# Lqm26/BMCNet-ESR

Measured on AMD Instinct MI355X. Metric: LR-voxel-frames/sec x4 SR train step, NFS-shaped 180x240 (BASELINE configs[1] / [2]), f32, higher is better.
Workload: dtype f32; 1 GPU; BMCNet(scale=4, n_c=128, n_b=5) x4 SR train step, NFS-shaped 180x240 (BASELINE configs[1] / [2]) -> 720x960, bs=4/GPU, arithmetic fp32 (native fp32 MFMA; 3x3 convolutions through Winograd F(4x4,3x3) / F(2x2,3x3) transforms in fp32), SEQL=9 SEQN=2 (8 windows BPTT), event scatter + fwd + MSE + bwd + Adam(amsgrad); global_batch=4, parallelism=dp1, rccl_ranks=1, rccl_initialised_before_headline_run=False

## Files before the change

### bmcnet-esr_amd/bmc_hip/ops.py

```python
from __future__ import annotations

import ctypes as C
import os
import threading
import weakref
from typing import List, Optional, Sequence

import torch

from . import lib

CK = 16
_cur_dev = torch._C._cuda_getDevice


_STREAM_OVERRIDE = None
_STREAM_OVERRIDE_TS = None


def _stream():
    if _STREAM_OVERRIDE is not None:
        return _STREAM_OVERRIDE
    return torch._C._cuda_getCurrentRawStream(_cur_dev())

# ... 302 lines not shown
    G, Cout, Cin, taps = w4.shape
    if wino:
        npos = 36 if wino == 4 else 16
        hit = _cache_get(spec, ("fw", npos), owner)
        if hit is not None:
            return hit
        cp = coutpad(Cout)
        out = torch.empty(G * spec.kpad * npos * cp, device=w4.device, dtype=torch.float32)
        fn, nm = (lib._pack_wino4, "bmc_pack_weight_wino4") if wino == 4 else (lib._pack_wino, "bmc_pack_weight_wino")
        lib.call(fn, nm, w4.data_ptr(), spec.kmap(w4.device).data_ptr(), G, Cout, Cin,
                 spec.kpad, cp, 0, 0, 0, out.data_ptr(), _stream())
        _cache_put(spec, ("fw", npos), owner, out)
        return out
    hit = _cache_get(spec, ("f", MATH), owner)
    if hit is not None:
        return hit
    cp = coutpad(Cout)
    out = torch.empty(G * spec.kpad * taps * cp, device=w4.device, dtype=torch.float32)
    lib.call(lib._pack_w, "bmc_pack_weight", w4.data_ptr(), spec.kmap(w4.device).data_ptr(), G, Cout, Cin, taps,
             spec.kpad, cp, out.data_ptr(), _stream())
    if MATH:
        out = _split_planes(out, cp)
    _cache_put(spec, ("f", MATH), owner, out)
    return out


def _packed_weight_t(w4: torch.Tensor, spec: ConvSpec, src_index: int, owner, wino=False):
    G, Cout, Cin, taps = w4.shape
    k0 = sum(spec.nch[:src_index])
    nk = spec.nch[src_index]
    nkpad = coutpad(nk)
    c16 = round_up(Cout, CK)
    if wino:
        npos = 36 if wino == 4 else 16
        hit = _cache_get(spec, ("tw", src_index, npos), owner)
        if hit is not None:
            return hit
        out = torch.empty(G * c16 * npos * nkpad, device=w4.device, dtype=torch.float32)
        fn, nm = (lib._pack_wino4, "bmc_pack_weight_wino4") if wino == 4 else (lib._pack_wino, "bmc_pack_weight_wino")
        lib.call(fn, nm, w4.data_ptr(), spec.kmap(w4.device).data_ptr(), G, Cout, Cin,
                 c16, nkpad, 1, k0, nk, out.data_ptr(), _stream())
        _cache_put(spec, ("tw", src_index, npos), owner, out)
        return out
    hit = _cache_get(spec, ("t", src_index, MATH), owner)
    if hit is not None:
        return hit
    out = torch.empty(G * c16 * taps * nkpad, device=w4.device, dtype=torch.float32)
    lib.call(lib._pack_wt, "bmc_pack_weight_t", w4.data_ptr(), spec.kmap(w4.device).data_ptr(), G, Cout, Cin, taps,
             k0, nk, nkpad, c16, out.data_ptr(), _stream())
    if MATH:
        out = _split_planes(out, nkpad)
    _cache_put(spec, ("t", src_index, MATH), owner, out)
    return out



def conv_raw(srcs: List[lib.Src], wpacked, w_group_stride, bias, bias_group_stride, out_ptr, out_batch_stride,
             out_pix_stride, B, H, W, Cout, taps, relu=False, residual: Optional[lib.Src] = None, bpg=None,
             accumulate=False, flops=0.0, mask: Optional[lib.Src] = None, wino=False):
    a = lib.ConvArgs()
    a.nsrc = len(srcs)
    for i, s in enumerate(srcs):
        a.src[i] = s
    a.wpacked = wpacked.data_ptr()
    a.bias = bias.data_ptr() if bias is not None else None
    a.w_group_stride = w_group_stride * MATH // 2 if MATH else w_group_stride
    a.math = MATH
    if wino:
        assert MATH == 0 and taps == 9
        a.w_group_stride = w_group_stride // 9 * (36 if wino == 4 else 16)
        a.math = 5 if wino == 4 else 4
    a.bias_group_stride = bias_group_stride
    a.batch_per_group = bpg if bpg else B
    a.out = out_ptr
    a.out_batch_stride = out_batch_stride
    a.out_pix_stride = out_pix_stride
    a.B, a.H, a.W = B, H, W
    a.Cout, a.Coutpad = Cout, coutpad(Cout)
    a.taps = taps
    a.relu = int(relu)
    a.residual = residual if residual is not None else _null_src()
    a.mask = mask if mask is not None else _null_src()
    a.accumulate = int(accumulate)
    e0 = _prof_begin()
    lib.call(lib._conv, "bmc_conv", C.byref(a), _stream())
    _prof_end(e0, ("wino4_conv<9,128>" if wino == 4 else "wino_conv<9,128>") if wino else
              "conv_kernel<%d,%d>" % (taps, 32 if a.Coutpad == 32 else 128), flops,
              4.0 * B * H * W * (sum(x.nch for x in srcs) + Cout * (1 + (residual is not None) + (mask is not None) + bool(accumulate))))
    if PROFILE is not None and e0 is not None:
        PROFILE_WINO[0 if wino else 1] += 1


_ZEROS = {}


def _zeros(device):
    z = _ZEROS.get(device)
    if z is None:
        z = torch.zeros(64, device=device, dtype=torch.float32)
        _ZEROS[device] = z
    return z


TAP_SPLIT_TILES = 8


def pgemm_raw(a_src: lib.Src, srcs: List[lib.Src], B, H, W, taps, bpg, M, N, device, flops=0.0, want_bias=False):
    G = B // bpg
    mpad, npad = round_up(M, 32), round_up(N, 32)
    if taps == 9:
        cols = 32 if MATH == 3 else 64
        n_nblk = (npad + cols - 1) // cols
        tiles = ((H + 3) // 4) * ((W + 15) // 16)
        target = 256
    else:
        n_nblk = (npad + 127) // 128
        tiles = (H * W + 63) // 64
        target = 256
    other = G * ((mpad + 127) // 128) * n_nblk
    nsplit = max(1, min(bpg * tiles, target // max(other, 1)))
    tap_groups = 1
    if taps == 9 and MATH in (0, 1) and bpg * tiles < TAP_SPLIT_TILES * nsplit and nsplit >= 3:
        tap_groups = 3
        nsplit = max(1, min(bpg * tiles, target // max(other * 3, 1)))
    slabs = torch.empty(nsplit * G * taps * mpad * npad, device=device, dtype=torch.float32)
    p = lib.PgemmArgs()
    p.a = a_src
    p.nsrc = len(srcs)
    for i, s in enumerate(srcs):
        p.src[i] = s
    p.B, p.H, p.W, p.taps = B, H, W, taps
    p.batch_per_group = bpg
    p.slabs = slabs.data_ptr()
    p.nsplit = nsplit
    p.zeros = _zeros(device).data_ptr()
    p.math = MATH
    p.tap_groups = tap_groups
    bslabs = None
    if want_bias:
        bslabs = torch.empty(nsplit * G * 4 * mpad, device=device, dtype=torch.float32)
        p.bias_slabs = bslabs.data_ptr()
    else:
        p.bias_slabs = None
    _on_side(slabs, bslabs)
    e0 = _prof_begin()
    lib.call(lib._pgemm, "bmc_pgemm", C.byref(p), _stream())
    _prof_end(e0, "pgemm_kernel<%d>" % taps, flops, 4.0 * B * H * W * (a_src.nch + sum(x.nch for x in srcs)) + 4.0 * slabs.numel())
    if want_bias:
        return slabs, nsplit, G, bslabs
    return slabs, nsplit, G


WINO_WGRAD = os.environ.get("BMC_WINO_WGRAD", "1") != "0"
WINO4_WGRAD = os.environ.get("BMC_WINO4_WGRAD", "0") != "0"
WINO4_WGRAD_MIN_STAGES = int(os.environ.get("BMC_WINO4_WGRAD_MIN_STAGES", 24))


def wgrad_wino4_ok(B, H, W):
    if not WINO4_WGRAD:
        return False
    stages = B * ((H + 3) // 4) * (((W + 3) // 4 + 3) // 4)
    return stages >= 32 * WINO4_WGRAD_MIN_STAGES


def wino_wgrad_ok(a_src, x_srcs, spec, taps, Cout, G):
    if not (WINO and WINO_WGRAD and MATH == 0 and taps == 9 and G == 1 and Cout == 128 and len(x_srcs) == 1 and spec.kpad == 128):
        return False
    xs = x_srcs[0]
    if not (xs.nch == 128 and xs.pix_stride == 128 and a_src.nch == 128 and a_src.pix_stride == 128):
        return False
    k0 = spec.kmap_host[0]
    return k0 >= 0 and spec.kmap_host == list(range(k0, k0 + 128))


WGRAD_MERGE = max(1, min(8, int(os.environ.get("BMC_WGRAD_MERGE", 5))))
WGRAD_MERGE_MAX_PIXELS = int(os.environ.get("BMC_WGRAD_MERGE_MAX_PIXELS", 1 << 17))


_WINDOW = [0]


def next_window():
    _WINDOW[0] += 1
    return _WINDOW[0]


def current_window():
    return _WINDOW[0]


class _MergeQueue:
    __slots__ = ("items", "spec", "dev", "w_param", "b_param", "want_bias", "k0", "full", "H", "W", "window", "pg")

    def __init__(self, spec, dev, w_param, b_param, want_bias, k0, full, H, W, window, pg=None):
        self.items = []
        self.spec, self.dev, self.w_param, self.b_param, self.want_bias, self.k0, self.full, self.H, self.W, self.window, self.pg = \
            spec, dev, w_param, b_param, want_bias, k0, full, H, W, window, pg


_MERGE = {}
_FLUSH_QUEUED = set()
PTR_TABLE_MAX = 256


def flush_wgrads(task=None):
    if task is None:
        task = torch._C._current_graph_task_id()
    _FLUSH_QUEUED.discard(task)
    qs = _MERGE.pop(task, None)
    if not qs:
        return
    for q in list(qs.values()):
        if q.items:
            _launch_merged(q)


def _queue_flush(task):
    if task not in _FLUSH_QUEUED:
        _FLUSH_QUEUED.add(task)
        torch.autograd.Variable._execution_engine.queue_callback(lambda: flush_wgrads(task))


_TABLES = {}


def _table_src(srcs, batches, btot, dev):
    ptrs = []
    for s_, nb in zip(srcs, batches):
        mod = s_.batch_mod if s_.batch_mod >= 1 else 1
        ptrs.extend(s_.ptr + 4 * (((i + s_.batch_shift) % mod) * s_.batch_stride) for i in range(nb))
    st = _stream()
    key = (dev.index, st.value if hasattr(st, "value") else st, tuple(ptrs))
    table = _TABLES.get(key)
    if table is None:
        if len(_TABLES) >= 8192:
            _TABLES.clear()
        table = torch.empty(btot, device=dev, dtype=torch.int64)
        lib.call(lib._ptr_table, "bmc_ptr_table", (C.c_ulonglong * btot)(*ptrs), btot, table.data_ptr(), st)
        if not torch.cuda.is_current_stream_capturing():
            _TABLES[key] = table
    t = lib.Src()
    t.ptr = table.data_ptr()
    t.batch_stride, t.pix_stride, t.nch, t.batch_shift, t.batch_mod = 0, srcs[0].pix_stride, srcs[0].nch, 0, -1
    return t, table


def _launch_merged(q):
    items, q.items = q.items, []
    keep = tuple(t for it in items for t in it[3])
    npx = items[0][2] * q.H * q.W
    if q.pg is not None:
        taps, Cout, w_shape = q.pg
        batches = [it[2] for it in items]
        btot = sum(batches)
        nx = len(items[0][1])
        with wgrad_side(npx, [q.w_param, q.b_param] if q.want_bias else [q.w_param], keep):
            a_t, tab_a = _table_src([it[0] for it in items], batches, btot, q.dev)
            x_tt = [_table_src([it[1][k] for it in items], batches, btot, q.dev) for k in range(nx)]
            x_t = [t for t, _ in x_tt]
            _on_side(tab_a, *[tb for _, tb in x_tt])
            r = pgemm_raw(a_t, x_t, btot, q.H, q.W, taps, btot, Cout, q.spec.kpad, q.dev,
                          flops=2.0 * btot * q.H * q.W * Cout * taps * q.spec.kreal, want_bias=q.want_bias)
            reduce_wgrad(r[0], r[1], 1, taps, Cout, q.spec, q.dev, r[3] if q.want_bias else None, q.w_param,
                         q.b_param if q.want_bias else None, w_shape)
        return
    with wgrad_side(npx, [q.w_param, q.b_param] if q.want_bias else [q.w_param], keep):
        _wgrad_wino([it[0] for it in items], [it[1] for it in items], [it[2] for it in items], q.H, q.W, q.spec, q.dev, q.w_param,
                    q.b_param, None, q.want_bias, q.k0, q.full)


def _queue_use(key, make_queue, item, task, npx):
    qs = _MERGE.setdefault(task, {})
    q = qs.get(key)
    if q is None or q.w_param is not item[4] or q.window != item[5]:
        if q is not None and q.items:
            _launch_merged(q)
        q = qs[key] = make_queue()
    if q.pg is not None and q.items and sum(it[2] for it in q.items) + item[2] > PTR_TABLE_MAX:
        _launch_merged(q)
    _queue_flush(task)
    _side_arm(npx)
    q.items.append(item[:4])
    if len(q.items) >= WGRAD_MERGE:
        _launch_merged(q)


def _mergeable(B, H, W, w_param, b_param, want_bias, keep, window):
    task = torch._C._current_graph_task_id()
    ok = (WGRAD_MERGE > 1 and window is not None and B * H * W <= WGRAD_MERGE_MAX_PIXELS and task >= 0 and w_param is not None
          and not isinstance(w_param, (tuple, list)) and is_sink(w_param) and (not want_bias or is_sink(b_param)) and keep
          and not torch.cuda.is_current_stream_capturing())
    return ok, task


def wgrad_pgemm(a_src, x_srcs, B, H, W, taps, Cout, spec, dev, w_param, b_param, w_shape, G=1, want_bias=True, keep=(), window=None):
    if G == 1:
        ok, task = _mergeable(B, H, W, w_param, b_param, want_bias, keep, window)
        if ok and B <= PTR_TABLE_MAX and all(x.batch_mod != -1 for x in x_srcs) and a_src.batch_mod != -1:
            key = (id(w_param), "pg", taps, len(x_srcs), H, W, bool(want_bias))
            _queue_use(key, lambda: _MergeQueue(spec, dev, w_param, b_param, want_bias, None, spec.covers_all, H, W, window,
                                                pg=(taps, Cout, w_shape)),
                       (a_src, list(x_srcs), B, tuple(keep), w_param, window), task, B * H * W)
            return None, None
    with wgrad_side(B * H * W, _flat_params(w_param, b_param if want_bias else None), keep):
        r = pgemm_raw(a_src, x_srcs, B, H, W, taps, B // G, Cout, spec.kpad, dev, flops=2.0 * B * H * W * Cout * taps * spec.kreal,
                      want_bias=want_bias)
        return reduce_wgrad(r[0], r[1], G, taps, Cout, spec, dev, r[3] if want_bias else None, w_param,
# ... 1056 lines not shown
```

### bmcnet-esr_amd/csrc/wino4_wgrad.hip

```cpp
#include "bmc_common.h"
#include "dma_ring.h"
#include <stdlib.h>

#ifndef BMC_W4G_ABL
#define BMC_W4G_ABL 0
#endif

#ifdef BMC_W4G_STAMP
__device__ unsigned long long g_w4g_stamp[8][64][8];
#define W4G_STAMP(it, k) do { if (blockIdx.x == 8 && (threadIdx.x & 63) == 0 && (it) >= 40 && (it) < 104) g_w4g_stamp[threadIdx.x >> 6][(it) - 40][(k)] = __builtin_amdgcn_s_memtime(); } while (0)
#else
#define W4G_STAMP(it, k) do { } while (0)
#endif

namespace {

struct Wgrad4K {
    SrcDev a;
    SrcDev x;
    int B, H, W;
    int TY, SX;
    int nstages, nsplit;
    float* part;
    float* bias_part;
};

typedef float f32x2 __attribute__((ext_vector_type(2)));

__device__ __forceinline__ const float* uni(const float* p) {
    const unsigned long long v = reinterpret_cast<unsigned long long>(p);
    const unsigned lo = __builtin_amdgcn_readfirstlane((unsigned)v), hi = __builtin_amdgcn_readfirstlane((unsigned)(v >> 32));
    return reinterpret_cast<const float*>(((unsigned long long)hi << 32) | lo);
}

constexpr int NPW = 18;
constexpr int TS = 4;
constexpr int CH = 64;
constexpr int PIMG = TS * CH;
constexpr int IMG = NPW * PIMG;
constexpr int SIMG = 2 * IMG;
constexpr int XPC = 23, YPC = 16;
constexpr int RAWX = XPC * 256;
constexpr int RAWF = (XPC + YPC) * 256;
constexpr int NPC = XPC + YPC;
constexpr int PPW = 10;
constexpr int LDSF = 2 * RAWF + 2 * SIMG;

template <int TG>
__device__ __forceinline__ void wgrad4_body(const Wgrad4K& a, float* const lds, const int split, const int chh, const int kh) {
    const int tid = threadIdx.x, lane = tid & 63;
    const int wave = __builtin_amdgcn_readfirstlane(tid >> 6);
    float* const rawb = lds;
    float* const imgb = lds + 2 * RAWF;
    const unsigned lds_raw = (unsigned)(size_t)(__attribute__((address_space(3))) void*)rawb;

    const int pg = wave >> 2, cb = (wave >> 1) & 1, kb = wave & 1;
    const int l31 = lane & 31, lh = lane >> 5;
    const int aoff = 3 * pg * PIMG + lh * CH + 32 * cb + l31;
    const int boff = IMG + 3 * pg * PIMG + lh * CH + 32 * kb + l31;
    f32x16 acc[9];
#pragma unroll
    for (int i = 0; i < 9; ++i)
#pragma unroll
        for (int r = 0; r < 16; ++r) acc[i][r] = 0.f;

    const bool requester = wave >= 4;
    unsigned poff[PPW];
    unsigned pla[PPW];
    unsigned pxm = 0;
    auto piece_of = [&](const int j) { return min((wave & 3) + 4 * j, NPC - 1); };
    auto slot_of = [&](const int p, int& r, int& c) __attribute__((always_inline)) {
        if (p < XPC) { const int q = 4 * p + (lane >> 4); r = q / 18; c = q - 18 * r; return q < 90; }
        const int q = 4 * (p - XPC) + (lane >> 4); r = q >> 4; c = q & 15;
        return true;
    };
#pragma unroll
    for (int j = 0; j < PPW; ++j) {
        const int p = piece_of(j);
        int r, c;
        const bool real = slot_of(p, r, c);
        poff[j] = real ? (unsigned)(((r * a.W + c) * 128 + (lane & 15) * 4) * 4) : 0u;
        pla[j] = lds_raw + (unsigned)(p * 1024);
        pxm |= p < XPC ? 1u << j : 0u;
    }
    unsigned zm = 0;
    static_assert(PPW <= 32, "zm is a bit mask");

    const int per_img = a.TY * a.SX;
    const int st0 = (int)((long long)a.nstages * split / a.nsplit), st1 = (int)((long long)a.nstages * (split + 1) / a.nsplit);
    int nb = st0 / per_img, nty, nsx;
    {
        const int r = st0 - nb * per_img;
        nty = r / a.SX; nsx = r - nty * a.SX;
    }
    nb = __builtin_amdgcn_readfirstlane(nb); nty = __builtin_amdgcn_readfirstlane(nty); nsx = __builtin_amdgcn_readfirstlane(nsx);
    const float* xbat = nullptr;
    const float* ybat = nullptr;
    const float* xrow = nullptr;
    const float* yrow = nullptr;
    bool rowborder = false;
    auto row_setup = [&]() __attribute__((always_inline)) {
        xbat = uni(src_batch_ptr(a.x, nb) + kh * CH);
        ybat = uni(src_batch_ptr(a.a, nb) + chh * CH);
        const int y0 = 4 * nty - 1 + TG;
        rowborder = y0 < 0 || y0 + 4 >= a.H;
        xrow = xbat + (long long)y0 * a.W * 128;
        yrow = ybat + (long long)(4 * nty) * a.W * 128;
    };
    row_setup();

    const float* rq_xs = nullptr;
    const float* rq_ys = nullptr;
    int rq_y0 = 0, rq_x0 = 0;
    unsigned rq_lo = 0;
    bool rq_border = false;
    auto rq_begin = [&](const int rb) __attribute__((always_inline)) {
        rq_lo = (unsigned)(rb * RAWF * 4);
        rq_y0 = 4 * nty - 1 + TG; rq_x0 = 16 * nsx - 1;
        rq_border = rowborder || nsx == 0 || rq_x0 + 17 >= a.W;
        rq_xs = rq_border ? xbat : xrow + rq_x0 * 128;
        rq_ys = rq_border ? ybat : yrow + (rq_x0 + 1) * 128;
        zm = 0;
        if (BMC_W4G_ABL & 16) return;
        if (++nsx == a.SX) {
            nsx = 0;
            if (++nty == a.TY) { nty = 0; ++nb; }
            row_setup();
        }
    };
    auto rq_piece = [&](const int j) __attribute__((always_inline)) {
        if (BMC_W4G_ABL & 2) return;
        unsigned o = poff[j];
        if (rq_border) {
            asm volatile("; image border" ::: "memory");
            const bool isx = (pxm >> j) & 1;
            int r, c;
            const bool real = slot_of(piece_of(j), r, c);
            const int y = (isx ? rq_y0 : rq_y0 + 1 - TG) + r, x = (isx ? rq_x0 : rq_x0 + 1) + c;
            const bool inside = y >= 0 && y < a.H && x >= 0 && x < a.W;
            const int yc = min(max(y, 0), a.H - 1), xc = min(max(x, 0), a.W - 1);
            o = real ? (unsigned)(((yc * a.W + xc) * 128 + (lane & 15) * 4) * 4) : 0u;
            zm |= (real && !inside) ? (1u << j) : 0u;
        }
        asm volatile("s_mov_b32 m0, %2\n\ts_nop 1\n\tglobal_load_lds_dwordx4 %0, %1" ::"v"(o), "s"(((pxm >> j) & 1) ? rq_xs : rq_ys),
                     "s"(pla[j] + rq_lo) : "memory");
    };
    auto patch = [&](const int rb) __attribute__((always_inline)) {
        if (__builtin_amdgcn_ballot_w64(zm != 0) == 0) return;
#pragma unroll
        for (int j = 0; j < PPW; ++j)
            if ((zm >> j) & 1) *reinterpret_cast<f32x4*>(rawb + (pla[j] - lds_raw) / 4 + rb * RAWF + lane * 4) = f32x4{0.f, 0.f, 0.f, 0.f};
    };

    const int cp = lane & 31;
    f32x2 bsum = {0.f, 0.f};
    auto xcols = [&](const f32x2 (&w)[6], float* const dst) __attribute__((always_inline)) {
        const f32x2 ta = w[4] - 4.f * w[2], tb = w[3] - 4.f * w[1], tc = w[4] - w[2], te = w[3] - w[1];
        *reinterpret_cast<f32x2*>(dst) = 4.f * w[0] - 5.f * w[2] + w[4];
        *reinterpret_cast<f32x2*>(dst + PIMG) = ta + tb;
        *reinterpret_cast<f32x2*>(dst + 2 * PIMG) = ta - tb;
        *reinterpret_cast<f32x2*>(dst + 3 * PIMG) = tc + 2.f * te;
        *reinterpret_cast<f32x2*>(dst + 4 * PIMG) = tc - 2.f * te;
        *reinterpret_cast<f32x2*>(dst + 5 * PIMG) = 4.f * w[1] - 5.f * w[3] + w[5];
    };
    auto ycols = [&](const f32x2 (&w)[4], float* const dst) __attribute__((always_inline)) -> f32x2 {
        const f32x2 s = w[0] + w[2], t = w[1] + w[3], p = w[0] + 4.f * w[2], q = w[1] + 4.f * w[3];
        const f32x2 m1 = s + t;
        *reinterpret_cast<f32x2*>(dst) = w[0];
        *reinterpret_cast<f32x2*>(dst + PIMG) = m1;
        *reinterpret_cast<f32x2*>(dst + 2 * PIMG) = s - t;
        *reinterpret_cast<f32x2*>(dst + 3 * PIMG) = p + 2.f * q;
        *reinterpret_cast<f32x2*>(dst + 4 * PIMG) = p - 2.f * q;
        *reinterpret_cast<f32x2*>(dst + 5 * PIMG) = w[3];
        return m1;
    };
    auto transform = [&](const float* const raw, float* const img) __attribute__((always_inline)) {
        if (BMC_W4G_ABL & 4) return;
        auto ld2 = [](const float* p) __attribute__((always_inline)) { return *reinterpret_cast<const f32x2*>(p); };
#pragma unroll
        for (int inst = 0; inst < 2; ++inst) {
            const int pt = 2 * inst + (lane >> 5);
            if (wave == 0) {
                const float* const s = raw + (4 * pt) * CH + 2 * cp;
                f32x2 d[3][6], w[6];
#pragma unroll
                for (int c = 0; c < 6; ++c)
#pragma unroll
                    for (int k = 0; k < 3; ++k) d[k][c] = ld2(s + (2 * k * 18 + c) * CH);
#pragma unroll
                for (int c = 0; c < 6; ++c) w[c] = 4.f * d[0][c] - 5.f * d[1][c] + d[2][c];
                xcols(w, img + IMG + ((TG == 0 ? 0 : 2) * 6) * PIMG + pt * CH + 2 * cp);
            } else if (wave < 3) {
                const float* const s = raw + ((1 - TG) * 18 + 4 * pt) * CH + 2 * cp;
                constexpr float al = TG == 0 ? -4.f : -1.f;
                const float ga = (TG == 0 ? 1.f : 2.f) * (wave == 2 ? -1.f : 1.f);
                f32x2 d[4][6], w[6];
#pragma unroll
                for (int c = 0; c < 6; ++c)
#pragma unroll
                    for (int k = 0; k < 4; ++k) d[k][c] = ld2(s + (k * 18 + c) * CH);
#pragma unroll
                for (int c = 0; c < 6; ++c) w[c] = (d[3][c] + al * d[1][c]) + ga * (d[2][c] + al * d[0][c]);
                xcols(w, img + IMG + (((TG == 0 ? 1 : 0) + (wave == 2 ? 1 : 0)) * 6) * PIMG + pt * CH + 2 * cp);
            } else {
                const float* const s = raw + RAWX + (4 * pt) * CH + 2 * cp;
                constexpr float ka = TG == 0 ? 1.f : 4.f, la = TG == 0 ? 1.f : 2.f;
                f32x2 y[4][4], u0[4], u1[4], u2[4];
#pragma unroll
                for (int c = 0; c < 4; ++c)
#pragma unroll
                    for (int k = 0; k < 4; ++k) y[k][c] = ld2(s + (16 * k + c) * CH);
#pragma unroll
                for (int c = 0; c < 4; ++c) {
                    const f32x2 p = y[0][c] + ka * y[2][c], q = y[1][c] + ka * y[3][c];
                    if (TG == 0) { u0[c] = y[0][c]; u1[c] = p + la * q; u2[c] = p - la * q; }
                    else { u0[c] = p + la * q; u1[c] = p - la * q; u2[c] = y[3][c]; }
                }
                float* const dd = img + pt * CH + 2 * cp;
                ycols(u0, dd);
                const f32x2 m11 = ycols(u1, dd + 6 * PIMG);
                ycols(u2, dd + 12 * PIMG);
                if (TG == 0) bsum += m11;
            }
            __builtin_amdgcn_sched_barrier(0);
        }
    };

    auto multiply = [&](const float* const img) __attribute__((always_inline)) {
        float af[3][2], bf[3][2];
        auto frag = [&](const int i) __attribute__((always_inline)) {
            const int u = i / 3, j = i - 3 * u, sl = i % 3;
#pragma unroll
            for (int ks = 0; ks < 2; ++ks) {
                if (BMC_W4G_ABL & 8) { af[sl][ks] = 1.f + ks; bf[sl][ks] = 2.f + j; asm volatile("" : "+v"(af[sl][ks]), "+v"(bf[sl][ks])); continue; }
                af[sl][ks] = img[aoff + (6 * u + j) * PIMG + 2 * ks * CH];
                bf[sl][ks] = img[boff + (6 * u + j) * PIMG + 2 * ks * CH];
            }
        };
        frag(0);
        frag(1);
#pragma unroll
        for (int i = 0; i < 9; ++i) {
            __builtin_amdgcn_sched_barrier(0);
            if (i + 2 < 9) frag(i + 2);
            __builtin_amdgcn_sched_barrier(0);
#pragma unroll
            for (int ks = 0; ks < 2; ++ks) {
                if (BMC_W4G_ABL & 1) acc[i][0] += af[i % 3][ks] * bf[i % 3][ks];
                else acc[i] = __builtin_amdgcn_mfma_f32_32x32x2f32(af[i % 3][ks], bf[i % 3][ks], acc[i], 0, 0, 0);
            }
        }
        __builtin_amdgcn_sched_barrier(0);
    };

    const int n = st1 - st0;
    if (n > 0) {
        rq_begin(0);
        if (requester) {
#pragma unroll
            for (int j = 0; j < PPW; ++j) rq_piece(j);
            dma_wait<0>();
            patch(0);
        }
        ring_publish();
        if (n > 1) {
            rq_begin(1);
            if (requester) {
#pragma unroll
                for (int j = 0; j < PPW; ++j) rq_piece(j);
            }
        }
        if (!requester) transform(rawb, imgb);
        dma_wait<0>();
        if (n > 1 && requester) patch(1);
        ring_publish();
    }
    for (int it = 0; it < n; ++it) {
        const float* const img = imgb + (it & 1) * SIMG;
        const bool req = it + 2 < n, more = it + 1 < n;
        W4G_STAMP(it, 0);
        if (req) rq_begin(it & 1);
        W4G_STAMP(it, 1);
        if (requester && req) {
#pragma unroll
            for (int j = 0; j < PPW; ++j) rq_piece(j);
        }
        W4G_STAMP(it, 2);
        __builtin_amdgcn_sched_barrier(0);
        multiply(img);
        __builtin_amdgcn_sched_barrier(0);
        W4G_STAMP(it, 3);
        if (!requester && more) transform(rawb + ((it + 1) & 1) * RAWF, imgb + ((it + 1) & 1) * SIMG);
        W4G_STAMP(it, 4);
        if (!(BMC_W4G_ABL & 32)) dma_wait<0>();
        W4G_STAMP(it, 5);
        if (requester && req) patch(it & 1);
        ring_publish();
        W4G_STAMP(it, 6);
    }

    {
        float* const P = a.part + ((((long long)split * 8 + (TG * 4 + chh * 2 + kh)) * 8 + wave) * 9) * 1024 + lane * 4;
#pragma unroll
        for (int i = 0; i < 9; ++i)
#pragma unroll
            for (int m = 0; m < 4; ++m)
                stg16(P + (i * 4 + m) * 256, f32x4{acc[i][4 * m], acc[i][4 * m + 1], acc[i][4 * m + 2], acc[i][4 * m + 3]});
    }
    if (TG == 0 && kh == 0 && a.bias_part) {
        if (wave == 3) *reinterpret_cast<f32x2*>(lds + (lane >> 5) * CH + 2 * cp) = bsum;
        __syncthreads();
        if (tid < CH) a.bias_part[(long long)split * 128 + 64 * chh + tid] = lds[tid] + lds[CH + tid];
    }
}

__global__ __launch_bounds__(512, 2) void wino4_wgrad_kernel(const Wgrad4K a) {
    __shared__ __attribute__((aligned(16))) float lds[LDSF];
    int type, split;
    if ((a.nsplit & 7) == 0) {
        const int j = blockIdx.x >> 3;
        type = j & 7; split = (j >> 3) * 8 + (blockIdx.x & 7);
    } else {
        type = blockIdx.x & 7; split = blockIdx.x >> 3;
    }
    const int chh = (type >> 1) & 1, kh = type & 1;
    if (type & 4) wgrad4_body<1>(a, lds, split, chh, kh);
    else wgrad4_body<0>(a, lds, split, chh, kh);
}

__global__ __launch_bounds__(256) void wino4_wgrad_reduce_kernel(const float* __restrict__ part, int nsplit, float* __restrict__ dw,
                                                                int ldw, int k0, int accumulate, const float* __restrict__ bias_part,
                                                                float* __restrict__ db) {
    __shared__ float red[8][36][32];
    const int ol = threadIdx.x & 31, pp = threadIdx.x >> 5;
    if ((int)blockIdx.y == 32) {
        if (blockIdx.x != 0) return;
        __shared__ float bs[2][128];
        const int cc = threadIdx.x & 127, hf = threadIdx.x >> 7;
        float s = 0.f;
        for (int i = hf; i < nsplit; i += 2) s += bias_part[(long long)i * 128 + cc];
        bs[hf][cc] = s;
        __syncthreads();
        if (hf == 0) {
            const float v = bs[0][cc] + bs[1][cc];
            db[cc] = accumulate ? db[cc] + v : v;
        }
        return;
    }
    const int co0 = 4 * blockIdx.y, ci = blockIdx.x * 32 + ol;
    const int chh = co0 >> 6, cb = (co0 >> 5) & 1, m = (co0 >> 3) & 3, lh = (co0 >> 2) & 1;
    const int kh = ci >> 6, kb = (ci >> 5) & 1;
    const float G[6][3] = {{0.25f, 0.f, 0.f}, {-1.f / 6, -1.f / 6, -1.f / 6}, {-1.f / 6, 1.f / 6, -1.f / 6},
                           {1.f / 24, 1.f / 12, 1.f / 6}, {1.f / 24, -1.f / 12, 1.f / 6}, {0.f, 0.f, 1.f}};
    f32x4 tap[9];
#pragma unroll
    for (int t = 0; t < 9; ++t) tap[t] = f32x4{0.f, 0.f, 0.f, 0.f};
    for (int p = pp; p < 36; p += 8) {
        const int xi = p / 6, nu = p - 6 * xi;
        const int type = (xi / 3) * 4 + chh * 2 + kh, wv = (nu / 3) * 4 + cb * 2 + kb, a9 = 3 * (xi % 3) + nu % 3;
        const float* ps = part + ((((long long)type * 8 + wv) * 9 + a9) * 4 + m) * 256 + (lh * 32 + ol) * 4;
        f32x4 u = {0.f, 0.f, 0.f, 0.f};
        for (int s = 0; s < nsplit; ++s) u += ldg16(ps + (long long)s * 36 * 16384);
#pragma unroll
        for (int i = 0; i < 3; ++i)
#pragma unroll
            for (int jj = 0; jj < 3; ++jj) tap[3 * i + jj] += (G[xi][i] * G[nu][jj]) * u;
    }
#pragma unroll
    for (int t = 0; t < 9; ++t)
#pragma unroll
        for (int e = 0; e < 4; ++e) red[pp][e * 9 + t][ol] = tap[t][e];
    __syncthreads();
    for (int q = pp; q < 36; q += 8) {
        float o = 0.f;
#pragma unroll
        for (int k = 0; k < 8; ++k) o += red[k][q][ol];
        const int e = q / 9, t = q - 9 * e;
        float* const d = dw + ((long long)(co0 + e) * ldw + k0 + ci) * 9 + t;
        *d = accumulate ? *d + o : o;
    }
}

}

#ifdef BMC_W4G_STAMP
extern "C" int bmc_w4g_read_stamps(unsigned long long* host) {
    return hipMemcpyFromSymbol(host, HIP_SYMBOL(g_w4g_stamp), sizeof(unsigned long long) * 8 * 64 * 8) == hipSuccess ? 0 : -1;
}
#endif

static long long w4g_stages(int B, int H, int W) { return (long long)B * ((H + 3) / 4) * (((W + 3) / 4 + TS - 1) / TS); }

extern "C" int bmc_wgrad_wino4_nsplit(int B, int H, int W) {
    if (B < 1 || H < 1 || W < 1) return 0;
    const long long stages = w4g_stages(B, H, W);
    const int per_type = bmc_num_cus() / 8 > 0 ? bmc_num_cus() / 8 : 1;
    return (int)(stages < per_type ? stages : per_type);
}

extern "C" int bmc_wgrad_wino4(const bmc_src_t* dy, const bmc_src_t* x, int B, int H, int W, int nsplit, float* part,
                               float* bias_part, bmc_stream_t s) {
    BMC_CHECK_ARG(dy && x && part && dy->ptr && x->ptr, "bmc_wgrad_wino4: null argument");
    BMC_CHECK_ARG(dy->nch == 128 && x->nch == 128, "bmc_wgrad_wino4: both operands must be 128-channel windows (got %d, %d)", dy->nch,
                  x->nch);
    BMC_CHECK_ARG(dy->pix_stride == 128 && x->pix_stride == 128, "bmc_wgrad_wino4: both operands must be dense in the channel axis "
                  "(pix_stride 128; got %d, %d)", dy->pix_stride, x->pix_stride);
    BMC_CHECK_ARG(B >= 1 && H >= 1 && W >= 1 && (long long)H * W * 128 < (1ll << 29), "bmc_wgrad_wino4: bad geometry");
    Wgrad4K k;
    k.a = to_dev(*dy); k.x = to_dev(*x);
    k.B = B; k.H = H; k.W = W;
    k.TY = (H + 3) / 4; k.SX = ((W + 3) / 4 + TS - 1) / TS;
    const long long stages = w4g_stages(B, H, W);
    BMC_CHECK_ARG(stages < (1ll << 31), "bmc_wgrad_wino4: too many tiles");
    BMC_CHECK_ARG(nsplit >= 1 && nsplit <= stages, "bmc_wgrad_wino4: nsplit must be in [1, %lld]", stages);
    k.nstages = (int)stages; k.nsplit = nsplit;
    k.part = part; k.bias_part = bias_part;
    hipLaunchKernelGGL(wino4_wgrad_kernel, dim3((unsigned)nsplit * 8), dim3(512), 0, (hipStream_t)s, k);
    BMC_CHECK_LAUNCH("bmc_wgrad_wino4");
    return 0;
}

extern "C" int bmc_wgrad_wino4_reduce(const float* part, int nsplit, float* dw, int ldw, int k0, int accumulate,
                                      const float* bias_part, float* db, bmc_stream_t s) {
    BMC_CHECK_ARG(part && dw && nsplit >= 1, "bmc_wgrad_wino4_reduce: bad arguments");
    BMC_CHECK_ARG(ldw >= 128 && k0 >= 0 && k0 + 128 <= ldw, "bmc_wgrad_wino4_reduce: columns [k0, k0 + 128) must lie inside the %d input "
                  "channels of the weight tensor", ldw);
    BMC_CHECK_ARG((bias_part == nullptr) == (db == nullptr), "bmc_wgrad_wino4_reduce: bias_part and db go together");
    hipLaunchKernelGGL(wino4_wgrad_reduce_kernel, dim3(4, bias_part ? 33 : 32), dim3(256), 0, (hipStream_t)s, part, nsplit, dw, ldw, k0,
                       accumulate, bias_part, db);
    BMC_CHECK_LAUNCH("bmc_wgrad_wino4_reduce");
    return 0;
}
```

Baseline: 44.44 LR-voxel-frames/s.

## Enable Winograd F(4x4) weight-gradient path with interleaved DMA/transform and new reduce

The F(4x4,3x3) Winograd weight-gradient kernel is now on by default. It is restructured so that all eight waves issue global-to-LDS loads and run the input transform, and both are spread across the MFMA sequence instead of being split between requester and transformer waves. The per-tile border offset math is hoisted into rq_begin. The reduction kernel is rewritten with one block per output group, unrolled split accumulation and an LDS inverse transform, to spread the reduction over more blocks. Making this path the default also risks slower or different numerics wherever it loses to the F(2x2) path it replaces.

New measurement: 46.64 LR-voxel-frames/s (median of 6 runs). +4.9%, better.

```diff
diff --git a/bmcnet-esr_amd/bmc_hip/ops.py b/bmcnet-esr_amd/bmc_hip/ops.py
--- a/bmcnet-esr_amd/bmc_hip/ops.py
+++ b/bmcnet-esr_amd/bmc_hip/ops.py
@@ -478,7 +478,7 @@
 
 
 WINO_WGRAD = os.environ.get("BMC_WINO_WGRAD", "1") != "0"
-WINO4_WGRAD = os.environ.get("BMC_WINO4_WGRAD", "0") != "0"
+WINO4_WGRAD = os.environ.get("BMC_WINO4_WGRAD", "1") != "0"
 WINO4_WGRAD_MIN_STAGES = int(os.environ.get("BMC_WINO4_WGRAD_MIN_STAGES", 24))
 
 
diff --git a/bmcnet-esr_amd/csrc/wino4_wgrad.hip b/bmcnet-esr_amd/csrc/wino4_wgrad.hip
--- a/bmcnet-esr_amd/csrc/wino4_wgrad.hip
+++ b/bmcnet-esr_amd/csrc/wino4_wgrad.hip
@@ -43,10 +43,33 @@
 constexpr int RAWX = XPC * 256;
 constexpr int RAWF = (XPC + YPC) * 256;
 constexpr int NPC = XPC + YPC;
-constexpr int PPW = 10;
+constexpr int PPW = 5;
 constexpr int LDSF = 2 * RAWF + 2 * SIMG;
-
-template <int TG>
+static_assert(LDSF * 4 <= 160 * 1024, "LDS budget");
+
+#ifndef BMC_W4G_MODE
+#define BMC_W4G_MODE 0
+#endif
+constexpr int dma_gap(const int j) {
+    return BMC_W4G_MODE == 1 ? 1 + 3 * j : (BMC_W4G_MODE == 2 ? j : (BMC_W4G_MODE == 3 ? 1 + 4 * j : 2 * j));
+}
+constexpr int TR_READ = 0, TR_COMB = 3, TR_OUT = 10;
+
+template <int I, int N>
+struct W4gFor {
+    template <class F>
+    static __device__ __forceinline__ void run(F&& f) {
+        f(std::integral_constant<int, I>{});
+        W4gFor<I + 1, N>::run(f);
+    }
+};
+template <int N>
+struct W4gFor<N, N> {
+    template <class F>
+    static __device__ __forceinline__ void run(F&&) {}
+};
+
+template <int TG, int ROLE>
 __device__ __forceinline__ void wgrad4_body(const Wgrad4K& a, float* const lds, const int split, const int chh, const int kh) {
     const int tid = threadIdx.x, lane = tid & 63;
     const int wave = __builtin_amdgcn_readfirstlane(tid >> 6);
@@ -64,11 +87,12 @@
 #pragma unroll
         for (int r = 0; r < 16; ++r) acc[i][r] = 0.f;
 
-    const bool requester = wave >= 4;
     unsigned poff[PPW];
+    unsigned pof[PPW];
     unsigned pla[PPW];
     unsigned pxm = 0;
-    auto piece_of = [&](const int j) { return min((wave & 3) + 4 * j, NPC - 1); };
+    auto piece_of = [&](const int j) { return min(wave + 8 * j, NPC - 1); };
+    const bool has_last = wave + 8 * (PPW - 1) < NPC;
     auto slot_of = [&](const int p, int& r, int& c) __attribute__((always_inline)) {
         if (p < XPC) { const int q = 4 * p + (lane >> 4); r = q / 18; c = q - 18 * r; return q < 90; }
         const int q = 4 * (p - XPC) + (lane >> 4); r = q >> 4; c = q & 15;
@@ -80,6 +104,7 @@
         int r, c;
         const bool real = slot_of(p, r, c);
         poff[j] = real ? (unsigned)(((r * a.W + c) * 128 + (lane & 15) * 4) * 4) : 0u;
+        pof[j] = poff[j];
         pla[j] = lds_raw + (unsigned)(p * 1024);
         pxm |= p < XPC ? 1u << j : 0u;
     }
@@ -111,16 +136,32 @@
 
     const float* rq_xs = nullptr;
     const float* rq_ys = nullptr;
-    int rq_y0 = 0, rq_x0 = 0;
     unsigned rq_lo = 0;
-    bool rq_border = false;
     auto rq_begin = [&](const int rb) __attribute__((always_inline)) {
         rq_lo = (unsigned)(rb * RAWF * 4);
-        rq_y0 = 4 * nty - 1 + TG; rq_x0 = 16 * nsx - 1;
-        rq_border = rowborder || nsx == 0 || rq_x0 + 17 >= a.W;
-        rq_xs = rq_border ? xbat : xrow + rq_x0 * 128;
-        rq_ys = rq_border ? ybat : yrow + (rq_x0 + 1) * 128;
+        const int y0 = 4 * nty - 1 + TG, x0 = 16 * nsx - 1;
+        const bool border = rowborder || nsx == 0 || x0 + 17 >= a.W;
+        rq_xs = border ? xbat : xrow + x0 * 128;
+        rq_ys = border ? ybat : yrow + (x0 + 1) * 128;
         zm = 0;
+        if (border) {
+            asm volatile("; image border" ::: "memory");
+#pragma unroll
+            for (int j = 0; j < PPW; ++j) {
+                const bool isx = (pxm >> j) & 1;
+                int r, c;
+                const bool real = slot_of(piece_of(j), r, c);
+                const int y = (isx ? y0 : y0 + 1 - TG) + r, x = (isx ? x0 : x0 + 1) + c;
+                const bool inside = y >= 0 && y < a.H && x >= 0 && x < a.W;
+                const int yc = min(max(y, 0), a.H - 1), xc = min(max(x, 0), a.W - 1);
+                pof[j] = real ? (unsigned)(((yc * a.W + xc) * 128 + (lane & 15) * 4) * 4) : 0u;
+                zm |= (real && !inside) ? (1u << j) : 0u;
+            }
+        } else {
+#pragma unroll
+            for (int j = 0; j < PPW; ++j) pof[j] = poff[j];
+        }
+        if (!has_last) zm &= ~(1u << (PPW - 1));
         if (BMC_W4G_ABL & 16) return;
         if (++nsx == a.SX) {
             nsx = 0;
@@ -130,19 +171,8 @@
     };
     auto rq_piece = [&](const int j) __attribute__((always_inline)) {
         if (BMC_W4G_ABL & 2) return;
-        unsigned o = poff[j];
-        if (rq_border) {
-            asm volatile("; image border" ::: "memory");
-            const bool isx = (pxm >> j) & 1;
-            int r, c;
-            const bool real = slot_of(piece_of(j), r, c);
-            const int y = (isx ? rq_y0 : rq_y0 + 1 - TG) + r, x = (isx ? rq_x0 : rq_x0 + 1) + c;
-            const bool inside = y >= 0 && y < a.H && x >= 0 && x < a.W;
-            const int yc = min(max(y, 0), a.H - 1), xc = min(max(x, 0), a.W - 1);
-            o = real ? (unsigned)(((yc * a.W + xc) * 128 + (lane & 15) * 4) * 4) : 0u;
-            zm |= (real && !inside) ? (1u << j) : 0u;
-        }
-        asm volatile("s_mov_b32 m0, %2\n\ts_nop 1\n\tglobal_load_lds_dwordx4 %0, %1" ::"v"(o), "s"(((pxm >> j) & 1) ? rq_xs : rq_ys),
+        if (j == PPW - 1 && !has_last) return;
+        asm volatile("s_mov_b32 m0, %2\n\ts_nop 1\n\tglobal_load_lds_dwordx4 %0, %1" ::"v"(pof[j]), "s"(((pxm >> j) & 1) ? rq_xs : rq_ys),
                      "s"(pla[j] + rq_lo) : "memory");
     };
     auto patch = [&](const int rb) __attribute__((always_inline)) {
@@ -152,81 +182,82 @@
             if ((zm >> j) & 1) *reinterpret_cast<f32x4*>(rawb + (pla[j] - lds_raw) / 4 + rb * RAWF + lane * 4) = f32x4{0.f, 0.f, 0.f, 0.f};
     };
 
-    const int cp = lane & 31;
+    const int pt = 2 * (wave >> 2) + (lane >> 5), cp = lane & 31;
+    constexpr int NK = ROLE == 0 ? 3 : 4;
+    constexpr int NC = ROLE == 3 ? 4 : 6;
+    constexpr int KS = ROLE == 0 ? 2 * 18 * CH : (ROLE == 3 ? 16 * CH : 18 * CH);
+    const int tsrc = (ROLE == 0 ? 4 * pt * CH : (ROLE == 3 ? RAWX + 4 * pt * CH : ((1 - TG) * 18 + 4 * pt) * CH)) + 2 * cp;
+    const int tdst = (ROLE == 3 ? 0 : IMG + (ROLE == 0 ? (TG == 0 ? 0 : 2) : (TG == 0 ? 1 : 0) + (ROLE == 2 ? 1 : 0)) * 6 * PIMG) + pt * CH + 2 * cp;
+    f32x2 td[NC][NK];
+    f32x2 tw[3][NC];
     f32x2 bsum = {0.f, 0.f};
-    auto xcols = [&](const f32x2 (&w)[6], float* const dst) __attribute__((always_inline)) {
-        const f32x2 ta = w[4] - 4.f * w[2], tb = w[3] - 4.f * w[1], tc = w[4] - w[2], te = w[3] - w[1];
-        *reinterpret_cast<f32x2*>(dst) = 4.f * w[0] - 5.f * w[2] + w[4];
-        *reinterpret_cast<f32x2*>(dst + PIMG) = ta + tb;
-        *reinterpret_cast<f32x2*>(dst + 2 * PIMG) = ta - tb;
-        *reinterpret_cast<f32x2*>(dst + 3 * PIMG) = tc + 2.f * te;
-        *reinterpret_cast<f32x2*>(dst + 4 * PIMG) = tc - 2.f * te;
-        *reinterpret_cast<f32x2*>(dst + 5 * PIMG) = 4.f * w[1] - 5.f * w[3] + w[5];
-    };
-    auto ycols = [&](const f32x2 (&w)[4], float* const dst) __attribute__((always_inline)) -> f32x2 {
-        const f32x2 s = w[0] + w[2], t = w[1] + w[3], p = w[0] + 4.f * w[2], q = w[1] + 4.f * w[3];
-        const f32x2 m1 = s + t;
-        *reinterpret_cast<f32x2*>(dst) = w[0];
-        *reinterpret_cast<f32x2*>(dst + PIMG) = m1;
-        *reinterpret_cast<f32x2*>(dst + 2 * PIMG) = s - t;
-        *reinterpret_cast<f32x2*>(dst + 3 * PIMG) = p + 2.f * q;
-        *reinterpret_cast<f32x2*>(dst + 4 * PIMG) = p - 2.f * q;
-        *reinterpret_cast<f32x2*>(dst + 5 * PIMG) = w[3];
-        return m1;
-    };
-    auto transform = [&](const float* const raw, float* const img) __attribute__((always_inline)) {
+    auto ld2 = [](const float* p) __attribute__((always_inline)) { return *reinterpret_cast<const f32x2*>(p); };
+    auto st2 = [](float* p, const f32x2 v) __attribute__((always_inline)) { *reinterpret_cast<f32x2*>(p) = v; };
+    auto tgap = [&](auto gc, const float* const raw, float* const img) __attribute__((always_inline)) {
+        constexpr int G = decltype(gc)::value;
         if (BMC_W4G_ABL & 4) return;
-        auto ld2 = [](const float* p) __attribute__((always_inline)) { return *reinterpret_cast<const f32x2*>(p); };
-#pragma unroll
-        for (int inst = 0; inst < 2; ++inst) {
-            const int pt = 2 * inst + (lane >> 5);
-            if (wave == 0) {
-                const float* const s = raw + (4 * pt) * CH + 2 * cp;
-                f32x2 d[3][6], w[6];
-#pragma unroll
-                for (int c = 0; c < 6; ++c)
-#pragma unroll
-                    for (int k = 0; k < 3; ++k) d[k][c] = ld2(s + (2 * k * 18 + c) * CH);
-#pragma unroll
-                for (int c = 0; c < 6; ++c) w[c] = 4.f * d[0][c] - 5.f * d[1][c] + d[2][c];
-                xcols(w, img + IMG + ((TG == 0 ? 0 : 2) * 6) * PIMG + pt * CH + 2 * cp);
-            } else if (wave < 3) {
-                const float* const s = raw + ((1 - TG) * 18 + 4 * pt) * CH + 2 * cp;
+        constexpr int cr = G - TR_READ, cc = G - TR_COMB;
+        if constexpr (cr >= 0 && cr < NC) {
+#pragma unroll
+            for (int k = 0; k < NK; ++k) td[cr][k] = ld2(raw + tsrc + k * KS + cr * CH);
+        }
+        if constexpr (cc >= 0 && cc < NC) {
+            const f32x2* const d = td[cc];
+            if constexpr (ROLE == 0) {
+                tw[0][cc] = 4.f * d[0] - 5.f * d[1] + d[2];
+            } else if constexpr (ROLE < 3) {
                 constexpr float al = TG == 0 ? -4.f : -1.f;
-                const float ga = (TG == 0 ? 1.f : 2.f) * (wave == 2 ? -1.f : 1.f);
-                f32x2 d[4][6], w[6];
-#pragma unroll
-                for (int c = 0; c < 6; ++c)
-#pragma unroll
-                    for (int k = 0; k < 4; ++k) d[k][c] = ld2(s + (k * 18 + c) * CH);
-#pragma unroll
-                for (int c = 0; c < 6; ++c) w[c] = (d[3][c] + al * d[1][c]) + ga * (d[2][c] + al * d[0][c]);
-                xcols(w, img + IMG + (((TG == 0 ? 1 : 0) + (wave == 2 ? 1 : 0)) * 6) * PIMG + pt * CH + 2 * cp);
+                constexpr float ga = (TG == 0 ? 1.f : 2.f) * (ROLE == 2 ? -1.f : 1.f);
+                tw[0][cc] = (d[3] + al * d[1]) + ga * (d[2] + al * d[0]);
             } else {
-                const float* const s = raw + RAWX + (4 * pt) * CH + 2 * cp;
                 constexpr float ka = TG == 0 ? 1.f : 4.f, la = TG == 0 ? 1.f : 2.f;
-                f32x2 y[4][4], u0[4], u1[4], u2[4];
-#pragma unroll
-                for (int c = 0; c < 4; ++c)
-#pragma unroll
-                    for (int k = 0; k < 4; ++k) y[k][c] = ld2(s + (16 * k + c) * CH);
-#pragma unroll
-                for (int c = 0; c < 4; ++c) {
-                    const f32x2 p = y[0][c] + ka * y[2][c], q = y[1][c] + ka * y[3][c];
-                    if (TG == 0) { u0[c] = y[0][c]; u1[c] = p + la * q; u2[c] = p - la * q; }
-                    else { u0[c] = p + la * q; u1[c] = p - la * q; u2[c] = y[3][c]; }
+                const f32x2 p = d[0] + ka * d[2], q = d[1] + ka * d[3];
+                if (TG == 0) { tw[0][cc] = d[0]; tw[1][cc] = p + la * q; tw[2][cc] = p - la * q; }
+                else { tw[0][cc] = p + la * q; tw[1][cc] = p - la * q; tw[2][cc] = d[3]; }
+            }
+        }
+        constexpr int ko = G - TR_OUT;
+        if constexpr (ko >= 0 && ko < 6 && (ko & 1) == 0) {
+            constexpr int k = ko >> 1;
+            if constexpr (ROLE < 3) {
+                const f32x2* const w = tw[0];
+                float* const dst = img + tdst;
+                if (k == 0) {
+                    st2(dst, 4.f * w[0] - 5.f * w[2] + w[4]);
+                    st2(dst + 5 * PIMG, 4.f * w[1] - 5.f * w[3] + w[5]);
+                } else if (k == 1) {
+                    const f32x2 ta = w[4] - 4.f * w[2], tb = w[3] - 4.f * w[1];
+                    st2(dst + PIMG, ta + tb);
+                    st2(dst + 2 * PIMG, ta - tb);
+                } else {
+                    const f32x2 tc = w[4] - w[2], te = w[3] - w[1];
+                    st2(dst + 3 * PIMG, tc + 2.f * te);
+                    st2(dst + 4 * PIMG, tc - 2.f * te);
                 }
-                float* const dd = img + pt * CH + 2 * cp;
-                ycols(u0, dd);
-                const f32x2 m11 = ycols(u1, dd + 6 * PIMG);
-                ycols(u2, dd + 12 * PIMG);
-                if (TG == 0) bsum += m11;
+            } else {
+                const f32x2* const w = tw[k];
+                float* const dst = img + tdst + 6 * k * PIMG;
+                const f32x2 s = w[0] + w[2], t = w[1] + w[3], p = w[0] + 4.f * w[2], q = w[1] + 4.f * w[3];
+                const f32x2 m1 = s + t;
+                st2(dst, w[0]);
+                st2(dst + PIMG, m1);
+                st2(dst + 2 * PIMG, s - t);
+                st2(dst + 3 * PIMG, p + 2.f * q);
+                st2(dst + 4 * PIMG, p - 2.f * q);
+                st2(dst + 5 * PIMG, w[3]);
+                if (TG == 0 && k == 1) bsum += m1;
             }
-            __builtin_amdgcn_sched_barrier(0);
-        }
-    };
-
-    auto multiply = [&](const float* const img) __attribute__((always_inline)) {
+        }
+    };
+
+    auto stage = [&](const int it, auto reqc, auto morec) __attribute__((always_inline)) {
+        constexpr bool REQ = decltype(reqc)::value, MORE = decltype(morec)::value;
+        const float* const img = imgb + (it & 1) * SIMG;
+        const float* const traw = rawb + ((it + 1) & 1) * RAWF;
+        float* const timg = imgb + ((it + 1) & 1) * SIMG;
+        W4G_STAMP(it, 0);
+        if (REQ) rq_begin(it & 1);
+        W4G_STAMP(it, 1);
         float af[3][2], bf[3][2];
         auto frag = [&](const int i) __attribute__((always_inline)) {
             const int u = i / 3, j = i - 3 * u, sl = i % 3;
@@ -237,67 +268,59 @@
                 bf[sl][ks] = img[boff + (6 * u + j) * PIMG + 2 * ks * CH];
             }
         };
+        __builtin_amdgcn_sched_barrier(0);
         frag(0);
         frag(1);
-#pragma unroll
-        for (int i = 0; i < 9; ++i) {
+        W4gFor<0, 9>::run([&](auto ic) __attribute__((always_inline)) {
+            constexpr int i = decltype(ic)::value;
             __builtin_amdgcn_sched_barrier(0);
             if (i + 2 < 9) frag(i + 2);
             __builtin_amdgcn_sched_barrier(0);
-#pragma unroll
-            for (int ks = 0; ks < 2; ++ks) {
+            W4gFor<0, 2>::run([&](auto kc) __attribute__((always_inline)) {
+                constexpr int ks = decltype(kc)::value, g = 2 * i + ks;
                 if (BMC_W4G_ABL & 1) acc[i][0] += af[i % 3][ks] * bf[i % 3][ks];
                 else acc[i] = __builtin_amdgcn_mfma_f32_32x32x2f32(af[i % 3][ks], bf[i % 3][ks], acc[i], 0, 0, 0);
-            }
-        }
-        __builtin_amdgcn_sched_barrier(0);
+                if (REQ) {
+#pragma unroll
+                    for (int j = 0; j < PPW; ++j)
+                        if (dma_gap(j) == g) rq_piece(j);
+                }
+                if (MORE) tgap(std::integral_constant<int, g>{}, traw, timg);
+                __builtin_amdgcn_sched_barrier(0);
+            });
+            if (i == 4) W4G_STAMP(it, 2);
+        });
+        W4G_STAMP(it, 3);
+        if (!(BMC_W4G_ABL & 32)) dma_wait<0>();
+        W4G_STAMP(it, 4);
+        if (REQ) patch(it & 1);
+        ring_publish();
+        W4G_STAMP(it, 5);
     };
 
     const int n = st1 - st0;
-    if (n > 0) {
-        rq_begin(0);
-        if (requester) {
-#pragma unroll
-            for (int j = 0; j < PPW; ++j) rq_piece(j);
-            dma_wait<0>();
-            patch(0);
-        }
-        ring_publish();
-        if (n > 1) {
-            rq_begin(1);
-            if (requester) {
-#pragma unroll
-                for (int j = 0; j < PPW; ++j) rq_piece(j);
-            }
-        }
-        if (!requester) transform(rawb, imgb);
-        dma_wait<0>();
-        if (n > 1 && requester) patch(1);
-        ring_publish();
-    }
-    for (int it = 0; it < n; ++it) {
-        const float* const img = imgb + (it & 1) * SIMG;
-        const bool req = it + 2 < n, more = it + 1 < n;
-        W4G_STAMP(it, 0);
-        if (req) rq_begin(it & 1);
-        W4G_STAMP(it, 1);
-        if (requester && req) {
-#pragma unroll
-            for (int j = 0; j < PPW; ++j) rq_piece(j);
-        }
-        W4G_STAMP(it, 2);
-        __builtin_amdgcn_sched_barrier(0);
-        multiply(img);
-        __builtin_amdgcn_sched_barrier(0);
-        W4G_STAMP(it, 3);
-        if (!requester && more) transform(rawb + ((it + 1) & 1) * RAWF, imgb + ((it + 1) & 1) * SIMG);
-        W4G_STAMP(it, 4);
-        if (!(BMC_W4G_ABL & 32)) dma_wait<0>();
-        W4G_STAMP(it, 5);
-        if (requester && req) patch(it & 1);
-        ring_publish();
-        W4G_STAMP(it, 6);
-    }
+    if (n <= 0) return;
+    rq_begin(0);
+#pragma unroll
+    for (int j = 0; j < PPW; ++j) rq_piece(j);
+    dma_wait<0>();
+    patch(0);
+    ring_publish();
+    if (n > 1) {
+        rq_begin(1);
+#pragma unroll
+        for (int j = 0; j < PPW; ++j) rq_piece(j);
+    }
+    W4gFor<0, 18>::run([&](auto gc) __attribute__((always_inline)) { tgap(gc, rawb, imgb); });
+    dma_wait<0>();
+    if (n > 1) patch(1);
+    ring_publish();
+    using T_ = std::true_type;
+    using F_ = std::false_type;
+    int it = 0;
+    for (; it + 2 < n; ++it) stage(it, T_{}, T_{});
+    if (it + 1 < n) stage(it++, F_{}, T_{});
+    stage(it, F_{}, F_{});
 
     {
         float* const P = a.part + ((((long long)split * 8 + (TG * 4 + chh * 2 + kh)) * 8 + wave) * 9) * 1024 + lane * 4;
@@ -308,9 +331,19 @@
                 stg16(P + (i * 4 + m) * 256, f32x4{acc[i][4 * m], acc[i][4 * m + 1], acc[i][4 * m + 2], acc[i][4 * m + 3]});
     }
     if (TG == 0 && kh == 0 && a.bias_part) {
-        if (wave == 3) *reinterpret_cast<f32x2*>(lds + (lane >> 5) * CH + 2 * cp) = bsum;
+        if (ROLE == 3) *reinterpret_cast<f32x2*>(lds + pt * CH + 2 * cp) = bsum;
         __syncthreads();
-        if (tid < CH) a.bias_part[(long long)split * 128 + 64 * chh + tid] = lds[tid] + lds[CH + tid];
+        if (tid < CH) a.bias_part[(long long)split * 128 + 64 * chh + tid] = (lds[tid] + lds[CH + tid]) + (lds[2 * CH + tid] + lds[3 * CH + tid]);
+    }
+}
+
+template <int TG>
+__device__ __forceinline__ void wgrad4_role(const Wgrad4K& a, float* const lds, const int split, const int chh, const int kh) {
+    switch (__builtin_amdgcn_readfirstlane(threadIdx.x >> 6) & 3) {
+        case 0: wgrad4_body<TG, 0>(a, lds, split, chh, kh); break;
+        case 1: wgrad4_body<TG, 1>(a, lds, split, chh, kh); break;
+        case 2: wgrad4_body<TG, 2>(a, lds, split, chh, kh); break;
+        default: wgrad4_body<TG, 3>(a, lds, split, chh, kh); break;
     }
 }
 
@@ -324,61 +357,73 @@
         type = blockIdx.x & 7; split = blockIdx.x >> 3;
     }
     const int chh = (type >> 1) & 1, kh = type & 1;
-    if (type & 4) wgrad4_body<1>(a, lds, split, chh, kh);
-    else wgrad4_body<0>(a, lds, split, chh, kh);
-}
-
-__global__ __launch_bounds__(256) void wino4_wgrad_reduce_kernel(const float* __restrict__ part, int nsplit, float* __restrict__ dw,
-                                                                int ldw, int k0, int accumulate, const float* __restrict__ bias_part,
-                                                                float* __restrict__ db) {
-    __shared__ float red[8][36][32];
-    const int ol = threadIdx.x & 31, pp = threadIdx.x >> 5;
-    if ((int)blockIdx.y == 32) {
-        if (blockIdx.x != 0) return;
-        __shared__ float bs[2][128];
-        const int cc = threadIdx.x & 127, hf = threadIdx.x >> 7;
+    if (type & 4) wgrad4_role<1>(a, lds, split, chh, kh);
+    else wgrad4_role<0>(a, lds, split, chh, kh);
+}
+
+constexpr int RED_THREADS = 288, RED_GROUPS = 512;
+__global__ __launch_bounds__(RED_THREADS) void wino4_wgrad_reduce_kernel(const float* __restrict__ part, int nsplit, float* __restrict__ dw,
+                                                                        int ldw, int k0, int accumulate, const float* __restrict__ bias_part,
+                                                                        float* __restrict__ db) {
+    constexpr long long SSTRIDE = 36ll * 16384;
+    const int t = threadIdx.x;
+    if ((int)blockIdx.x == RED_GROUPS) {
+        if (t >= 128) return;
         float s = 0.f;
-        for (int i = hf; i < nsplit; i += 2) s += bias_part[(long long)i * 128 + cc];
-        bs[hf][cc] = s;
-        __syncthreads();
-        if (hf == 0) {
-            const float v = bs[0][cc] + bs[1][cc];
-            db[cc] = accumulate ? db[cc] + v : v;
-        }
+        int i = 0;
+        for (; i + 8 <= nsplit; i += 8) {
+            float q[8];
+#pragma unroll
+            for (int k = 0; k < 8; ++k) q[k] = bias_part[(long long)(i + k) * 128 + t];
+#pragma unroll
+            for (int k = 0; k < 8; ++k) s += q[k];
+        }
+        for (; i < nsplit; ++i) s += bias_part[(long long)i * 128 + t];
+        db[t] = accumulate ? db[t] + s : s;
         return;
     }
-    const int co0 = 4 * blockIdx.y, ci = blockIdx.x * 32 + ol;
-    const int chh = co0 >> 6, cb = (co0 >> 5) & 1, m = (co0 >> 3) & 3, lh = (co0 >> 2) & 1;
-    const int kh = ci >> 6, kb = (ci >> 5) & 1;
+    __shared__ f32x4 U[36][8];
+    const int c = blockIdx.x >> 5, r = blockIdx.x & 31;
+    const int chh = c >> 3, kh = (c >> 2) & 1, cb = (c >> 1) & 1, kb = c & 1;
+    const int m = r >> 3, lane0 = 8 * (r & 7);
+    {
+        const int p = t >> 3, qi = t & 7;
+        const int xi = p / 6, nu = p - 6 * xi;
+        const int type = (xi / 3) * 4 + chh * 2 + kh, wv = (nu / 3) * 4 + cb * 2 + kb, a9 = 3 * (xi % 3) + nu % 3;
+        const float* const ps = part + (((long long)type * 8 + wv) * 9 + a9) * 1024 + m * 256 + (lane0 + qi) * 4;
+        f32x4 u = {0.f, 0.f, 0.f, 0.f};
+        int s = 0;
+        for (; s + 8 <= nsplit; s += 8) {
+            f32x4 q[8];
+#pragma unroll
+            for (int k = 0; k < 8; ++k) q[k] = ldg16(ps + (s + k) * SSTRIDE);
+#pragma unroll
+            for (int k = 0; k < 8; ++k) u += q[k];
+        }
+        for (; s < nsplit; ++s) u += ldg16(ps + s * SSTRIDE);
+        U[p][qi] = u;
+    }
+    __syncthreads();
     const float G[6][3] = {{0.25f, 0.f, 0.f}, {-1.f / 6, -1.f / 6, -1.f / 6}, {-1.f / 6, 1.f / 6, -1.f / 6},
                            {1.f / 24, 1.f / 12, 1.f / 6}, {1.f / 24, -1.f / 12, 1.f / 6}, {0.f, 0.f, 1.f}};
-    f32x4 tap[9];
-#pragma unroll
-    for (int t = 0; t < 9; ++t) tap[t] = f32x4{0.f, 0.f, 0.f, 0.f};
-    for (int p = pp; p < 36; p += 8) {
-        const int xi = p / 6, nu = p - 6 * xi;
-        const int type = (xi / 3) * 4 + chh * 2 + kh, wv = (nu / 3) * 4 + cb * 2 + kb, a9 = 3 * (xi % 3) + nu % 3;
-        const float* ps = part + ((((long long)type * 8 + wv) * 9 + a9) * 4 + m) * 256 + (lh * 32 + ol) * 4;
-        f32x4 u = {0.f, 0.f, 0.f, 0.f};
-        for (int s = 0; s < nsplit; ++s) u += ldg16(ps + (long long)s * 36 * 16384);
-#pragma unroll
-        for (int i = 0; i < 3; ++i)
-#pragma unroll
-            for (int jj = 0; jj < 3; ++jj) tap[3 * i + jj] += (G[xi][i] * G[nu][jj]) * u;
-    }
-#pragma unroll
-    for (int t = 0; t < 9; ++t)
-#pragma unroll
-        for (int e = 0; e < 4; ++e) red[pp][e * 9 + t][ol] = tap[t][e];
-    __syncthreads();
-    for (int q = pp; q < 36; q += 8) {
-        float o = 0.f;
-#pragma unroll
-        for (int k = 0; k < 8; ++k) o += red[k][q][ol];
-        const int e = q / 9, t = q - 9 * e;
-        float* const d = dw + ((long long)(co0 + e) * ldw + k0 + ci) * 9 + t;
-        *d = accumulate ? *d + o : o;
-    }
+    const int e = t / 72, r2 = t - 72 * e, qi = r2 / 9, tap = r2 - 9 * qi, ti = tap / 3, tj = tap - 3 * ti;
+    float o = 0.f;
+#pragma unroll
+    for (int k = 0; k < 8; ++k) {
+        float tk = 0.f;
+#pragma unroll
+        for (int p = k; p < 36; p += 8) {
+            const int xi = p / 6, nu = p - 6 * xi;
+            float gi = 0.f, gj = 0.f;
+#pragma unroll
+            for (int q = 0; q < 3; ++q) { gi = q == ti ? G[xi][q] : gi; gj = q == tj ? G[nu][q] : gj; }
+            tk += (gi * gj) * U[p][qi][e];
+        }
+        o += tk;
+    }
+    const int co = 64 * chh + 32 * cb + 8 * m + 4 * (lane0 >> 5) + e, ci = 64 * kh + 32 * kb + (lane0 & 31) + qi;
+    float* const d = dw + ((long long)co * ldw + k0 + ci) * 9 + tap;
+    *d = accumulate ? *d + o : o;
 }
 
 }
@@ -426,7 +471,7 @@
     BMC_CHECK_ARG(ldw >= 128 && k0 >= 0 && k0 + 128 <= ldw, "bmc_wgrad_wino4_reduce: columns [k0, k0 + 128) must lie inside the %d input "
                   "channels of the weight tensor", ldw);
     BMC_CHECK_ARG((bias_part == nullptr) == (db == nullptr), "bmc_wgrad_wino4_reduce: bias_part and db go together");
-    hipLaunchKernelGGL(wino4_wgrad_reduce_kernel, dim3(4, bias_part ? 33 : 32), dim3(256), 0, (hipStream_t)s, part, nsplit, dw, ldw, k0,
+    hipLaunchKernelGGL(wino4_wgrad_reduce_kernel, dim3(RED_GROUPS + (bias_part ? 1 : 0)), dim3(RED_THREADS), 0, (hipStream_t)s, part, nsplit, dw, ldw, k0,
                        accumulate, bias_part, db);
     BMC_CHECK_LAUNCH("bmc_wgrad_wino4_reduce");
     return 0;
```
